# mrinmoy-iitg/SM_HPSS_MTL

Hardware: AMD Instinct MI355X
Metric: clips/sec HPSS+MTL-CNN fwd (1s@16kHz) (higher is better)
Workload: dtype f32

## Files before the change

sm_hpss_mtl_amd/build.py:

```python
from __future__ import annotations

import os
import subprocess
import sys
from concurrent.futures import ThreadPoolExecutor

HERE = os.path.dirname(os.path.abspath(__file__))
CSRC = os.path.join(HERE, "csrc")
OBJ = os.path.join(CSRC, "build")
LIB = os.path.join(HERE, "libsmh.so")
ARCH = "gfx950"
FLAGS = ["--offload-arch=" + ARCH, "-O3", "-fPIC", "-std=c++17", "-Wall", "-Wno-unused-function"]
EXTRA_FLAGS = {"smh_median_split.hip": ["-fno-honor-nans"], "smh_train.hip": ["-munsafe-fp-atomics"],
               "smh_tcn.hip": ["-fno-honor-nans"], "smh_tcn_bf16.hip": ["-fno-honor-nans"],
               "smh_train_bf16.hip": ["-munsafe-fp-atomics", "-fno-honor-nans"]}


def _sources():
    return sorted(f for f in os.listdir(CSRC) if f.endswith(".hip"))


def _headers_mtime():
    hs = [os.path.join(CSRC, f) for f in os.listdir(CSRC) if f.endswith(".h")]
    hs.append(os.path.join(HERE, "..", "include", "smh.h"))
    return max(os.path.getmtime(h) for h in hs)


LAB = False


def _compile(src: str, force: bool) -> str:
    obj = os.path.join(OBJ, src[:-4] + ".o")
    srcp = os.path.join(CSRC, src)
    if not force and os.path.exists(obj) and os.path.getmtime(obj) >= max(os.path.getmtime(srcp), _headers_mtime()):
        return obj
    cmd = ["hipcc", *FLAGS, *(["-DSMH_LAB"] if LAB else []), *EXTRA_FLAGS.get(src, []), "-c", srcp, "-o", obj]
    r = subprocess.run(cmd, capture_output=True, text=True)
    if r.returncode != 0:
        raise RuntimeError("hipcc failed for %s:\n%s\n%s" % (src, r.stdout, r.stderr))
    return obj


def build(force: bool = False, verbose: bool = True) -> str:
    os.makedirs(OBJ, exist_ok=True)
    srcs = _sources()
    with ThreadPoolExecutor(max_workers=min(6, len(srcs))) as ex:
        objs = list(ex.map(lambda s: _compile(s, force), srcs))
    if force or not os.path.exists(LIB) or any(os.path.getmtime(o) > os.path.getmtime(LIB) for o in objs):
        cmd = ["hipcc", "--offload-arch=" + ARCH, "-shared", "-fPIC", "-o", LIB, *objs]
        r = subprocess.run(cmd, capture_output=True, text=True)
        if r.returncode != 0:
            raise RuntimeError("link failed:\n%s\n%s" % (r.stdout, r.stderr))
    if verbose:
        print("built", LIB, "from", len(srcs), "HIP sources")
    return LIB


if __name__ == "__main__":
    LAB = "--lab" in sys.argv
    build(force="--force" in sys.argv or LAB)
```

sm_hpss_mtl_amd/csrc/smh_median.hip:

```cpp
#include <cstdlib>

#include "smh_median_kernel.h"
#include "smh_median_split.h"

namespace smh_median {

const Entry kPairs[] = {
    SMH_MEDIAN_E2(21, 11) SMH_MEDIAN_E2(17, 17)
    SMH_MEDIAN_E2(11, 11) SMH_MEDIAN_E2(11, 21) SMH_MEDIAN_E2(11, 31) SMH_MEDIAN_E2(11, 41) SMH_MEDIAN_E2(11, 51)
    SMH_MEDIAN_E2(21, 21) SMH_MEDIAN_E2(21, 31) SMH_MEDIAN_E2(21, 41) SMH_MEDIAN_E2(21, 51)
    SMH_MEDIAN_E2(31, 11) SMH_MEDIAN_E2(31, 21) SMH_MEDIAN_E2(31, 31) SMH_MEDIAN_E2(31, 41) SMH_MEDIAN_E2(31, 51)
    SMH_MEDIAN_E2(41, 11) SMH_MEDIAN_E2(41, 21) SMH_MEDIAN_E2(41, 31) SMH_MEDIAN_E2(41, 41) SMH_MEDIAN_E2(41, 51)
    SMH_MEDIAN_E2(51, 11) SMH_MEDIAN_E2(51, 21) SMH_MEDIAN_E2(51, 31) SMH_MEDIAN_E2(51, 41) SMH_MEDIAN_E2(51, 51)};

KernelFn find_pair_kernel(int lh, int lp) {
    for (const Entry &e : kPairs)
        if (e.lh == lh && e.lp == lp) return e.fn;
    return nullptr;
}

}

namespace {

// ... 93 lines not shown
    int bh = 0, bp = 0;
    for (int nsh = lh ? 1 : 0; nsh <= (lh ? 4 : 0); ++nsh) {
        if (lh && nsh > 1 && nt < 2 * lh * nsh) break;
        for (int nsp = lp ? 1 : 0; nsp <= (lp ? 6 : 0); ++nsp) {
            if (lp && nsp > 1 && K < 2 * lp * nsp) break;
            if (waves(K, nsh) + waves(nt, nsp) > maxwaves) continue;
            const long ch = lh ? (long)((nt + nsh - 1) / nsh + lh) * (lh + 6) : 0;
            const long cp = lp ? (long)((K + nsp - 1) / nsp + lp) * (lp + 6) : 0;
            const long c = ch > cp ? ch : cp;
            if (best < 0 || c < best) best = c, bh = nsh, bp = nsp;
        }
    }
    if (best < 0) return false;
    if (const char *ev = getenv("SMH_MEDIAN_SEG")) {
        int a = 0, b = 0;
        if (sscanf(ev, "%d,%d", &a, &b) == 2 && (!lh || a >= 1) && (!lp || b >= 1) &&
            waves(K, lh ? a : 0) + waves(nt, lp ? b : 0) <= maxwaves)
            bh = lh ? a : 0, bp = lp ? b : 0;
    }
    p->nsh = bh, p->nsp = bp, p->nwh = waves(K, bh), p->nwp = waves(nt, bp);
    return true;
}

int launch_small(const float *S, int B, int K, int T, int w, int along_t, float *out, hipStream_t st) {
    const size_t total = (size_t)B * K * T;
    const int bs = 256;
    hipLaunchKernelGGL(median_small_kernel, dim3((unsigned)((total + bs - 1) / bs)), dim3(bs), 0, st, S, out, K, T, w,
                       along_t, total);
    return smh::launch_status("median_small_kernel");
}

enum Family { kFamCopy = 0, kFamSmall = 1, kFamSplit = 2, kFamPersist = 3, kFamDeleteInsert = 4, kFamTwoSingles = 5 };
struct Route {
    int family, layout;
    Plan plan;
    KernelFn fn;
    const SplitEntry *se;
    const PersistEntry *pe;
    int n_cu;
};

int launch_route(int B, int K, int T, int lh, int lp, int harm_tmajor, Route *r) {
    *r = Route{};
    r->layout = harm_tmajor;
    r->fn = (lh && lp) ? find_pair_kernel(lh, lp) : find_single_kernel(lh, lp);
    if (!r->fn) return smh::set_error(SMH_E_INVALID, "no median kernel for (l_harm,l_perc)=(%d,%d)", lh, lp);
    Plan p;
    int rc = make_plan(K, T, lh, lp, &p);
    if (rc) return rc;
    static const bool no_split = getenv("SMH_MEDIAN_NOSPLIT") != nullptr;
    bool want_persist = (lh > 17 || lp > 17);
    if (const char *ev = getenv("SMH_MEDIAN_PERSIST")) want_persist = atoi(ev) != 0;
    int pthreads = 512;
    if (const char *ev = getenv("SMH_MEDIAN_PTHREADS")) pthreads = atoi(ev);
    if (const PersistEntry *pe = (no_split || !want_persist || !(lh && lp)) ? nullptr : find_persist_kernel(lh, lp, pthreads)) {
        static int n_cu = 0;
        if (n_cu == 0) {
            int dev = 0;
            SMH_CHECK_HIP(hipGetDevice(&dev));
            SMH_CHECK_HIP(hipDeviceGetAttribute(&n_cu, hipDeviceAttributeMultiprocessorCount, dev));
        }
        const int tile_bytes = persist_tile_bytes(K, T);
        const int g = T & 63;
        const bool conflict_free = (T & 1) || (g % 4 == 2);
        Plan q = p;
        if (p.ntiles == 1 && conflict_free && 2 * tile_bytes <= smh::kLdsBytesPerCU && B >= 2 * n_cu &&
            make_split_roles(K, T, lh, lp, pe->threads / 64, &q)) {
            r->family = kFamPersist, r->plan = q, r->pe = pe, r->n_cu = n_cu;
            return SMH_OK;
        }
    }
    if (const SplitEntry *se = no_split ? nullptr : find_split_kernel(lh, lp)) {
        Plan q = p;
        if (make_split_roles(K, p.TT, lh, lp, se->threads / 64, &q)) {
            r->family = kFamSplit, r->plan = q, r->se = se;
            return SMH_OK;
        }
    }
    if (harm_tmajor == 2) r->layout = 1;
    r->family = kFamDeleteInsert, r->plan = p;
    return SMH_OK;
}

int launch_routed(const Route &r, const float *S, int B, int K, int T, float *harm, float *perc, hipStream_t st) {
    if (r.family == kFamPersist) {
        const Plan &q = r.plan;
        const int lds = 2 * persist_tile_bytes(K, T);
        SMH_CHECK_HIP(hipFuncSetAttribute((const void *)r.pe->fn, hipFuncAttributeMaxDynamicSharedMemorySize, lds));
        hipLaunchKernelGGL(r.pe->fn, dim3(r.n_cu), dim3((q.nwh + q.nwp) * 64), lds, st, S, harm, perc, B, K, T, q.nsh,
                           q.nsp, q.nwh, r.layout);
        return smh::launch_status("hpss_median_persist_kernel");
    }
    if (r.family == kFamSplit) {
        const Plan &q = r.plan;
        SMH_CHECK_HIP(hipFuncSetAttribute((const void *)r.se->fn, hipFuncAttributeMaxDynamicSharedMemorySize, (int)q.lds));
        SMH_CHECK_HIP(hipFuncSetAttribute((const void *)r.se->fn_dma, hipFuncAttributeMaxDynamicSharedMemorySize, (int)q.lds));
        dim3 grid(q.ntiles, B), block((q.nwh + q.nwp) * 64);
        const bool probe_noload = smh::probe_env("SMH_MEDIAN_PROBE_NOLOAD") != nullptr;
        const char *ev = getenv("SMH_MEDIAN_DMA_STAGE");
        const size_t clip_bytes = (size_t)K * T * sizeof(float);
        const uintptr_t s0 = reinterpret_cast<uintptr_t>(S);
        const size_t align = (s0 % 16 == 0 && clip_bytes % 16 == 0) ? 16 : (s0 % 8 == 0 && clip_bytes % 8 == 0) ? 8 : 4;
        const bool dma = !(ev && atoi(ev) == 0) && !probe_noload && q.ntiles == 1 && q.TT >= T && s0 % 4 == 0 &&
                         ((T & 1) || ((T & 63) % 4 == 2)) && dma_stage_bytes(clip_bytes, align) <= q.lds;
        hipLaunchKernelGGL(dma ? r.se->fn_dma : r.se->fn, grid, block, q.lds, st, S, harm, perc, K, T, q.TT, dma ? T : q.stride, q.nsh,
                           q.nsp, q.nwh, r.layout, probe_noload ? 1.f : -__builtin_inff(), __builtin_inff(), nullptr, nullptr, 0);
        return smh::launch_status("hpss_median_split_kernel");
    }
    const Plan &p = r.plan;
    SMH_CHECK_HIP(hipFuncSetAttribute((const void *)r.fn, hipFuncAttributeMaxDynamicSharedMemorySize, (int)p.lds));
    dim3 grid(p.ntiles, B), block((p.nwh + p.nwp) * 64);
    hipLaunchKernelGGL(r.fn, grid, block, p.lds, st, S, harm, perc, K, T, p.TT, p.stride, p.nsh, p.nsp, p.nwh,
                       r.layout, -__builtin_inff(), __builtin_inff());
    return smh::launch_status("hpss_median_kernel");
}

int launch(const float *S, int B, int K, int T, int lh, int lp, float *harm, float *perc, hipStream_t st,
           int harm_tmajor = 0, int *written = nullptr) {
    if (written) *written = harm_tmajor;
    Route r;
    int rc = launch_route(B, K, T, lh, lp, harm_tmajor, &r);
    if (rc) return rc;
    if (written) *written = r.layout;
    return launch_routed(r, S, B, K, T, harm, perc, st);
}

int check_args(const void *S, int B, int K, int T, int w, const char *name) {
    SMH_REQUIRE(S != nullptr || B == 0, "%s: null input", name);
    SMH_REQUIRE(B >= 0 && K >= 1 && T >= 1, "%s: bad shape B=%d K=%d T=%d", name, B, K, T);
    SMH_REQUIRE(w >= 1 && w <= SMH_MAX_MEDIAN && (w & 1), "%s: window must be odd in [1,%d], got %d", name,
                SMH_MAX_MEDIAN, w);
    SMH_REQUIRE(B <= 65535, "%s: B=%d exceeds the grid limit; split the batch", name, B);
    return SMH_OK;
}

bool fast_ok(int n, int w) { return w >= 3 && w / 2 + 4 < n; }

bool pair_fused(int K, int T, int lh, int lp) { return fast_ok(T, lh) && fast_ok(K, lp) && find_pair_kernel(lh, lp); }

int hpss_route(int B, int K, int T, int lh, int lp, int want_tmajor, Route *r) {
    if (pair_fused(K, T, lh, lp)) return launch_route(B, K, T, lh, lp, want_tmajor, r);
    *r = Route{};
    r->family = kFamTwoSingles;
    return SMH_OK;
}

int time_route(int B, int K, int T, int lh, Route *r) {
    if (lh == 1 || !fast_ok(T, lh)) {
        *r = Route{};
        r->family = lh == 1 ? kFamCopy : kFamSmall;
        return SMH_OK;
    }
    return launch_route(B, K, T, lh, 0, 0, r);
}

int time_ex_route(int B, int K, int T, int lh, int harm_layout, Route *r) {
    if (lh == 1 || !fast_ok(T, lh) || harm_layout == 0) return time_route(B, K, T, lh, r);
    return launch_route(B, K, T, lh, 0, harm_layout, r);
}

}

namespace smh_median {
int rag_tile_frames(int K, int lh, int lp, int *stride) {
    static const bool no_split = getenv("SMH_MEDIAN_NOSPLIT") != nullptr;
    if (no_split || !(lh && lp) || !find_split_kernel(lh, lp)) return 0;
    const int hh = lh / 2;
    const int budget_words = (smh::kLdsBytesPerCU / 2 - 1024) / 4;
    int maxcols = budget_words / K;
    if ((maxcols & 1) == 0) maxcols -= 1;
    int TT = (maxcols - 2 * hh) & ~3;
    if (TT < 2 * hh + 8) return 0;
    if (stride) *stride = (TT + 2 * hh) | 1;
    return TT;
}

int launch_rag(const float *d_S, float *d_harm, float *d_perc, int K, int lh, int lp, const smh_rag::Clip *d_clips,
               const smh_rag::Item *d_items, int n_items, hipStream_t st) {
    if (n_items <= 0) return SMH_OK;
    int stride = 0;
    const int TT = rag_tile_frames(K, lh, lp, &stride);
    const SplitEntry *se = TT ? find_split_kernel(lh, lp) : nullptr;
    Plan q;
    if (!se || !make_split_roles(K, TT, lh, lp, se->threads / 64, &q))
        return smh::set_error(SMH_E_INVALID, "ragged medians: no block-split kernel for (l_harm,l_perc)=(%d,%d), K=%d", lh, lp, K);
    const size_t lds = (size_t)K * stride * sizeof(float);
    SMH_CHECK_HIP(hipFuncSetAttribute((const void *)se->fn, hipFuncAttributeMaxDynamicSharedMemorySize, (int)lds));
    const unsigned grid = (unsigned)(8 * (((long long)n_items + 7) / 8));
    hipLaunchKernelGGL(se->fn, dim3(grid), dim3((q.nwh + q.nwp) * 64), lds, st, d_S, d_harm, d_perc, K, 0, TT, stride, q.nsh, q.nsp,
                       q.nwh, 2, -__builtin_inff(), __builtin_inff(), d_clips, d_items, n_items);
    return smh::launch_status("hpss_median_split_kernel (ragged)");
}

int launch_hpss(const float *S, int B, int K, int T, int lh, int lp, float *harm, float *perc, int want_tmajor,
                hipStream_t st) {
    Route r;
    int rc = hpss_route(B, K, T, lh, lp, want_tmajor, &r);
    if (rc) return rc;
    rc = r.family == kFamTwoSingles ? smh_hpss_median_f32(nullptr, S, B, K, T, lh, lp, harm, perc, (void *)st)
                                    : launch_routed(r, S, B, K, T, harm, perc, st);
    return rc ? rc : r.layout;
}

bool blocked_harm_ok(int K, int T, int lh, int lp) {
    static const bool no_split = getenv("SMH_MEDIAN_NOSPLIT") != nullptr;
    if (no_split || !pair_fused(K, T, lh, lp)) return false;
    const SplitEntry *se = find_split_kernel(lh, lp);
    Plan p, q;
    return se && make_plan(K, T, lh, lp, &p) == SMH_OK && make_split_roles(K, p.TT, lh, lp, se->threads / 64, &q);
}
}

extern "C" int smh_median_time_f32(const smh_ctx *, const float *d_S, int B, int K, int T, int l_harm, float *d_harm,
                                   void *stream) {
    int rc = check_args(d_S, B, K, T, l_harm, "smh_median_time_f32");
    if (rc) return rc;
    SMH_REQUIRE(d_harm || B == 0, "smh_median_time_f32: null output");
    if (B == 0) return SMH_OK;
    hipStream_t st = (hipStream_t)stream;
    Route r;
    rc = time_route(B, K, T, l_harm, &r);
    if (rc) return rc;
    if (r.family == kFamCopy) {
        SMH_CHECK_HIP(hipMemcpyAsync(d_harm, d_S, (size_t)B * K * T * sizeof(float), hipMemcpyDeviceToDevice, st));
        return SMH_OK;
    }
    if (r.family == kFamSmall) return launch_small(d_S, B, K, T, l_harm, 1, d_harm, st);
    return launch_routed(r, d_S, B, K, T, d_harm, nullptr, st);
}

extern "C" int smh_median_time_ex_f32(const smh_ctx *, const float *d_S, int B, int K, int T, int l_harm, float *d_harm,
                                      int harm_layout, void *stream) {
    int rc = check_args(d_S, B, K, T, l_harm, "smh_median_time_ex_f32");
    if (rc) return rc;
    SMH_REQUIRE(harm_layout >= 0 && harm_layout <= 2, "smh_median_time_ex_f32: harm_layout must be 0, 1 or 2");
    SMH_REQUIRE(d_harm || B == 0, "smh_median_time_ex_f32: null output");
    if (B == 0) return harm_layout;
    Route r;
    rc = time_ex_route(B, K, T, l_harm, harm_layout, &r);
    if (rc) return rc;
    if (r.family == kFamCopy || r.family == kFamSmall) {
        rc = smh_median_time_f32(nullptr, d_S, B, K, T, l_harm, d_harm, stream);
        return rc ? rc : 0;
    }
    rc = launch_routed(r, d_S, B, K, T, d_harm, nullptr, (hipStream_t)stream);
    return rc ? rc : r.layout;
}

extern "C" int smh_median_freq_f32(const smh_ctx *, const float *d_S, int B, int K, int T, int l_perc, float *d_perc,
                                   void *stream) {
    int rc = check_args(d_S, B, K, T, l_perc, "smh_median_freq_f32");
    if (rc) return rc;
    SMH_REQUIRE(d_perc || B == 0, "smh_median_freq_f32: null output");
    if (B == 0) return SMH_OK;
    hipStream_t st = (hipStream_t)stream;
    if (l_perc == 1) {
        SMH_CHECK_HIP(hipMemcpyAsync(d_perc, d_S, (size_t)B * K * T * sizeof(float), hipMemcpyDeviceToDevice, st));
        return SMH_OK;
    }
    if (!fast_ok(K, l_perc)) return launch_small(d_S, B, K, T, l_perc, 0, d_perc, st);
    return launch(d_S, B, K, T, 0, l_perc, nullptr, d_perc, st);
}

extern "C" int smh_hpss_median_f32(const smh_ctx *, const float *d_S, int B, int K, int T, int l_harm, int l_perc,
                                   float *d_harm, float *d_perc, void *stream) {
    int rc = check_args(d_S, B, K, T, l_harm, "smh_hpss_median_f32");
    if (rc) return rc;
    rc = check_args(d_S, B, K, T, l_perc, "smh_hpss_median_f32");
    if (rc) return rc;
    SMH_REQUIRE((d_harm && d_perc) || B == 0, "smh_hpss_median_f32: null output");
    if (B == 0) return SMH_OK;
    Route r;
// ... 45 lines not shown
```

sm_hpss_mtl_amd/csrc/smh_median_split.h:

```cpp
#pragma once
#include <cstdint>
#include <type_traits>
#include <utility>

#include "smh_median_kernel.h"
#include "smh_rag.h"

namespace smh_median {

template <int W>
struct SplitTraits {
    static constexpr int H = W / 2;
    static constexpr int lo(int s) { return s - H - 1 > 0 ? s - H - 1 : 0; }
    static constexpr int hi(int s) { return s - 1 < H ? s - 1 : H; }
    static constexpr int off(int s) {
        int o = 0;
        for (int r = 1; r < s; ++r) o += hi(r) - lo(r) + 1;
        return o;
    }
    static constexpr int HIST = off(W);
};

template <int B, int E, typename F>
__device__ __forceinline__ void static_for(F &&f) {
    if constexpr (B < E) {
        f(std::integral_constant<int, B>{});
        static_for<B + 1, E>(f);
    }
}
template <int B, int E, typename F>
__device__ __forceinline__ void static_for_down(F &&f) {
    if constexpr (B < E) {
        f(std::integral_constant<int, E - 1>{});
        static_for_down<B, E - 1>(f);
    }
}

template <bool HasBelow, bool HasAbove>
__device__ __forceinline__ float insert_slot(float below, float x, float above) {
    if constexpr (HasBelow && HasAbove) return med3(below, x, above);
    else if constexpr (HasBelow) return fmaxf(below, x);
    else if constexpr (HasAbove) return fminf(x, above);
    else return x;
}

template <int W>
__device__ __forceinline__ void build_history(const float (&e)[W], float (&h)[SplitTraits<W>::HIST]) {
    using Tr = SplitTraits<W>;
    static_for<1, W>([&](auto sc) {
        constexpr int s = decltype(sc)::value;
        const float x = e[W - s];
        static_for<Tr::lo(s), Tr::hi(s) + 1>([&](auto ic) {
            constexpr int i = decltype(ic)::value;
            constexpr bool has_below = i - 1 >= 0;
            constexpr bool has_above = i <= s - 2;
            constexpr int po = Tr::off(s > 1 ? s - 1 : 1), pl = Tr::lo(s > 1 ? s - 1 : 1);
            const float below = has_below ? h[has_below ? po + (i - 1) - pl : 0] : 0.f;
            const float above = has_above ? h[has_above ? po + i - pl : 0] : 0.f;
            h[Tr::off(s) + i - Tr::lo(s)] = insert_slot<has_below, has_above>(below, x, above);
        });
    });
}

template <int W, int ES, int STORE>
__device__ __forceinline__ void split_median_walk(const float *line, int es_rt, int p0, int n_out, int n_steps, int n,
                                                  char *obase, unsigned boff, unsigned ostep) {
    using Tr = SplitTraits<W>;
    constexpr int H = W / 2;
    const int es = ES > 0 ? ES : es_rt;
    float e[W];
    float h[Tr::HIST];
    float pre[H + 1];

    const int plast = p0 + n_out - 1 + H;
    auto load_block = [&](int q0) {
        const int lo = p0 - H + q0;
        const bool interior = (lo >= 0) & (lo + W <= n) & (lo + W - 1 <= plast);
        if (__all(interior)) {
            const float *src = line + lo * es;
            static_for<0, W>([&](auto uc) { e[decltype(uc)::value] = src[decltype(uc)::value * es]; });
        } else {
            static_for<0, W>([&](auto uc) {
                const int pos = min(lo + decltype(uc)::value, plast);
                e[decltype(uc)::value] = line[reflect_hi(reflect_lo(pos), n) * es];
            });
        }
    };
    unsigned off = boff;
    auto emit = [&](int j, float v, bool guard) {
        if (!guard || j < n_out) {
            float *dst = reinterpret_cast<float *>(obase + off);
#ifdef SMH_NT_STORES
            if constexpr (STORE == kStridedStream) __builtin_nontemporal_store(v, dst);
            else *dst = v;
#else
            *dst = v;
#endif
        }
        off += ostep;
    };
    int n_min = n_out;
#pragma unroll
    for (int o = 32; o >= 1; o >>= 1) n_min = min(n_min, __shfl_xor(n_min, o, 64));

    auto forward = [&](auto fast_c, int j0) {
        constexpr bool FAST = decltype(fast_c)::value;
        static_for<0, W>([&](auto pc) {
            constexpr int p = decltype(pc)::value;
            constexpr int b = p + 1, a = W - 1 - p;
            {
                static_for_down<Tr::lo(b), Tr::hi(b) + 1>([&](auto ic) {
                    constexpr int i = decltype(ic)::value;
                    constexpr bool has_below = i - 1 >= 0;
                    constexpr bool has_above = i <= b - 2;
                    const float below = has_below ? pre[has_below ? i - 1 : 0] : 0.f;
                    const float above = has_above ? pre[i] : 0.f;
                    pre[i] = insert_slot<has_below, has_above>(below, e[p], above);
                });
                constexpr int i_lo = (H + 1 - b) > 0 ? (H + 1 - b) : 0;
                constexpr int i_hi = a < H + 1 ? a : H + 1;
                constexpr int ao = Tr::off(a > 0 ? a : 1), al = Tr::lo(a > 0 ? a : 1);
                float r = 0.f;
                static_for<i_lo, i_hi + 1>([&](auto ic) {
                    constexpr int i = decltype(ic)::value;
                    float t;
                    if constexpr (i == 0) t = pre[H];
                    else if constexpr (H - i < 0) t = h[ao + (i - 1) - al];
                    else t = fmaxf(h[ao + (i - 1) - al], pre[H - i]);
                    r = (i == i_lo) ? t : fminf(r, t);
                });
                emit(j0 + p, r, !FAST);
            }
        });
    };

    load_block(0);
    build_history<W>(e, h);
    {
        constexpr int po = Tr::off(W - 1), pl = Tr::lo(W - 1);
        emit(0, med3(h[po + (H - 1) - pl], e[0], h[po + H - pl]), false);
    }
    for (int j0 = 1; j0 < n_steps; j0 += W) {
        load_block(j0 + W - 1);
        if (j0 + W <= n_min) forward(std::true_type{}, j0);
        else forward(std::false_type{}, j0);
        if (j0 + W < n_steps) build_history<W>(e, h);
    }
}

template <int W>
__device__ __forceinline__ void build_history_b(const float (&e)[W - 1], float (&h)[SplitTraits<W>::HIST]) {
    using Tr = SplitTraits<W>;
    static_for<1, W>([&](auto sc) {
        constexpr int s = decltype(sc)::value;
        const float x = e[W - 1 - s];
        static_for<Tr::lo(s), Tr::hi(s) + 1>([&](auto ic) {
            constexpr int i = decltype(ic)::value;
            constexpr bool has_below = i - 1 >= 0;
            constexpr bool has_above = i <= s - 2;
            constexpr int po = Tr::off(s > 1 ? s - 1 : 1), pl = Tr::lo(s > 1 ? s - 1 : 1);
            const float below = has_below ? h[has_below ? po + (i - 1) - pl : 0] : 0.f;
            const float above = has_above ? h[has_above ? po + i - pl : 0] : 0.f;
            h[Tr::off(s) + i - Tr::lo(s)] = insert_slot<has_below, has_above>(below, x, above);
        });
    });
}

template <int W, int ES>
__device__ __forceinline__ void split_median_walk_blocked(const float *line, int p0, int n_out, int n_steps, int n,
                                                          char *obase, unsigned gk16, unsigned kofs) {
    using Tr = SplitTraits<W>;
    constexpr int H = W / 2, BK = W - 1;
    float e[BK];
    float h[Tr::HIST];
    float pre[H + 1];
    const int plast = p0 + n_out - 1 + H;
    auto load_block = [&](int q0) {
        const int lo = p0 - H + q0;
        const bool interior = (lo >= 0) & (lo + BK <= n) & (lo + BK - 1 <= plast);
        if (__all(interior)) {
            const float *src = line + lo * ES;
            static_for<0, BK>([&](auto uc) { e[decltype(uc)::value] = src[decltype(uc)::value * ES]; });
        } else {
            static_for<0, BK>([&](auto uc) {
                const int pos = min(lo + decltype(uc)::value, plast);
                e[decltype(uc)::value] = line[reflect_hi(reflect_lo(pos), n) * ES];
            });
        }
    };
    load_block(0);
    build_history_b<W>(e, h);
    for (int j0 = 0; j0 < n_steps; j0 += BK) {
        load_block(j0 + BK);
        float o4[4];
        static_for<0, BK>([&](auto pc) {
            constexpr int p = decltype(pc)::value;
            constexpr int b = p + 1, a = BK - p;
            static_for_down<Tr::lo(b), Tr::hi(b) + 1>([&](auto ic) {
                constexpr int i = decltype(ic)::value;
                constexpr bool has_below = i - 1 >= 0;
                constexpr bool has_above = i <= b - 2;
                const float below = has_below ? pre[has_below ? i - 1 : 0] : 0.f;
                const float above = has_above ? pre[i] : 0.f;
                pre[i] = insert_slot<has_below, has_above>(below, e[p], above);
            });
            constexpr int i_lo = (H + 1 - b) > 0 ? (H + 1 - b) : 0;
            constexpr int i_hi = a < H + 1 ? a : H + 1;
            constexpr int ao = Tr::off(a), al = Tr::lo(a);
            float r = 0.f;
            static_for<i_lo, i_hi + 1>([&](auto ic) {
                constexpr int i = decltype(ic)::value;
                float t;
                if constexpr (i == 0) t = pre[H];
                else if constexpr (H - i < 0) t = h[ao + (i - 1) - al];
                else t = fmaxf(h[ao + (i - 1) - al], pre[H - i]);
                r = (i == i_lo) ? t : fminf(r, t);
            });
            o4[p & 3] = r;
            if constexpr ((p & 3) == 3 || p == BK - 1) {
                constexpr int cnt = (p & 3) + 1, pf = p - (p & 3);
                const int j = j0 + pf, t = p0 + j;
                char *dst = obase + (unsigned)(t >> 4) * gk16 + kofs + (unsigned)(t & 15) * 4u;
                if (cnt == 4 && (t & 3) == 0 && j + 3 < n_out) {
                    float4u v = {o4[0], o4[1], o4[2], o4[3]};
                    *reinterpret_cast<float4u *>(dst) = v;
                } else {
#pragma unroll
                    for (int c = 0; c < cnt; ++c) {
                        const int tc = t + c;
                        if (j + c < n_out)
                            *reinterpret_cast<float *>(obase + (unsigned)(tc >> 4) * gk16 + kofs + (unsigned)(tc & 15) * 4u) = o4[c];
                    }
                }
            }
        });
        if (j0 + BK < n_steps) build_history_b<W>(e, h);
    }
}

__device__ __forceinline__ int stage_clip_dma(const char *src, int bytes, char *dst, int wave, int nwaves, int lane) {
    const int mis = (int)(reinterpret_cast<uintptr_t>(src) & 15);
    src -= mis;
    const int nchunks = (bytes + mis + 15) >> 4;
    for (int i = wave; i * 64 < nchunks; i += nwaves) {
        const int c = i * 64 + lane;
        if (c < nchunks)
            __builtin_amdgcn_global_load_lds(
                (const __attribute__((address_space(1))) void *)(src + (size_t)c * 16),
                (__attribute__((address_space(3))) void *)(dst + i * 1024), 16, 0, 0);
    }
    return mis;
}
__host__ __device__ constexpr size_t dma_stage_bytes(size_t bytes, size_t align) { return (bytes + (16 - align) + 15) & ~(size_t)15; }

template <int LH, int LP>
struct SplitCfg {
    static constexpr int kMaxW = LH > LP ? LH : LP;
    static constexpr int kThreads = kMaxW <= 17 ? 512 : 384;
    static constexpr int kWavesPerSimd = kMaxW <= 17 ? 4 : 3;
    static constexpr int kFlatBatch = kMaxW <= 17 ? 20 : 27;
};

template <int LH, int LP, bool DMA = false>
__global__ void __launch_bounds__((SplitCfg<LH, LP>::kThreads), (SplitCfg<LH, LP>::kWavesPerSimd))
hpss_median_split_kernel(const float *__restrict__ S, float *__restrict__ harm, float *__restrict__ perc, int K, int T,
                         int TT, int stride, int nsh, int nsp, int nwh, int harm_tmajor, float probe, float,
                         const smh_rag::Clip *__restrict__ rag, const smh_rag::Item *__restrict__ items, int n_items) {
    extern __shared__ __attribute__((aligned(16))) float tile_lds[];
    const float *tile = tile_lds;
    constexpr int HH = LH / 2;
    int b = blockIdx.y, tile_i = blockIdx.x;
    size_t spec_off, harm_off;
    if (rag) {
        const unsigned total = (unsigned)n_items, per_xcd = (total + 7u) >> 3;
        const unsigned j = blockIdx.x >> 3, n = (blockIdx.x & 7u) * per_xcd + j;
        if (j >= per_xcd || n >= total) return;
        const smh_rag::Item item = items[n];
        b = item.clip, tile_i = item.tile;
        T = rag[b].T;
        spec_off = (size_t)rag[b].spec_off, harm_off = (size_t)rag[b].harm_off;
    } else {
        spec_off = (size_t)b * K * T;
        harm_off = harm_tmajor == 2 ? (size_t)b * ((T + 15) >> 4) * K * 16 : spec_off;
    }
    const int t0 = tile_i * TT;
    const int t1 = min(T, t0 + TT);
    const int c0 = max(0, t0 - HH), c1 = min(T, t1 + HH);
    const int ncols = c1 - c0;
    const float *Sb = S + spec_off;
    const int wave = threadIdx.x >> 6, lane = threadIdx.x & 63;
    const int nwaves = blockDim.x >> 6;

    constexpr int kFlatBatch = SplitCfg<LH, LP>::kFlatBatch;
    if constexpr (DMA) {
        const int mis = stage_clip_dma(reinterpret_cast<const char *>(Sb), K * T * 4, reinterpret_cast<char *>(tile_lds), wave, nwaves, lane);
        tile = reinterpret_cast<const float *>(reinterpret_cast<const char *>(tile_lds) + mis);
        asm volatile("s_waitcnt vmcnt(0)" ::: "memory");
    } else if (probe > 0.f) {
        for (int i = threadIdx.x; i < K * stride; i += blockDim.x) tile_lds[i] = (float)((i * 2654435761u) >> 8) * (1.0f / 16777216.f);
    } else if (TT >= T && ((K * T) & 1) == 0 && K * T <= kFlatBatch * 2 * (int)blockDim.x) {
        const int n2 = (K * T) >> 1;
        const float2v *src = reinterpret_cast<const float2v *>(Sb);
        const unsigned magic = 0xFFFFFFFFu / (unsigned)T + 1u;
        const int extra = stride - T;
        float2v v[kFlatBatch];
#pragma unroll
        for (int r = 0; r < kFlatBatch; ++r) {
            const int idx = r * (int)blockDim.x + (int)threadIdx.x;
            v[r] = __builtin_nontemporal_load(src + min(idx, n2 - 1));
        }
#pragma unroll
        for (int r = 0; r < kFlatBatch; ++r) {
            const int idx = r * (int)blockDim.x + (int)threadIdx.x;
            if (idx < n2) {
                const unsigned g = 2u * (unsigned)idx;
                const unsigned k0 = __umulhi(g, magic), k1 = __umulhi(g + 1u, magic);
                tile_lds[g + k0 * extra] = v[r].x;
                tile_lds[g + 1u + k1 * extra] = v[r].y;
            }
        }
    } else if (((T | c0 | ncols) & 1) == 0 && ncols <= 128) {
        constexpr int kRowBatch = 6;
        const int n2 = ncols >> 1;
        for (int k0 = wave; k0 < K; k0 += nwaves * kRowBatch) {
            float2v v[kRowBatch];
#pragma unroll
            for (int r = 0; r < kRowBatch; ++r) {
                const int k = min(k0 + r * nwaves, K - 1);
                v[r] = __builtin_nontemporal_load(reinterpret_cast<const float2v *>(Sb + (size_t)k * T + c0) +
                                                  min(lane, n2 - 1));
            }
#pragma unroll
            for (int r = 0; r < kRowBatch; ++r) {
                const int k = k0 + r * nwaves;
                if (k < K && lane < n2) {
                    tile_lds[k * stride + 2 * lane] = v[r].x;
                    tile_lds[k * stride + 2 * lane + 1] = v[r].y;
                }
            }
        }
    } else {
        constexpr int kRowBatch = 6;
        for (int k0 = wave; k0 < K; k0 += nwaves * kRowBatch) {
            for (int cb = 0; cb < ncols; cb += 64) {
                float v[kRowBatch];
                const int c = cb + lane;
#pragma unroll
                for (int r = 0; r < kRowBatch; ++r) {
                    const int k = min(k0 + r * nwaves, K - 1);
                    v[r] = __builtin_nontemporal_load(Sb + (size_t)k * T + c0 + min(c, ncols - 1));
                }
#pragma unroll
                for (int r = 0; r < kRowBatch; ++r) {
                    const int k = k0 + r * nwaves;
                    if (k < K && c < ncols) tile_lds[k * stride + c] = v[r];
                }
            }
        }
    }
    __syncthreads();

    const int nt = t1 - t0;
    if (wave < nwh) {
        if constexpr (LH > 0) {
            const int id = wave * 64 + lane;
            if (id < K * nsh) {
                const int sg = id / K, k = id - sg * K;
                const int seglen = (nt + nsh - 1) / nsh;
                const int ts = t0 + sg * seglen;
                const int te = min(t1, ts + seglen);
                if (ts < te) {
                    const float *row = tile + k * stride - c0;
                    char *ob = reinterpret_cast<char *>(harm + harm_off);
                    if (harm_tmajor == 2)
                        split_median_walk_blocked<LH, 1>(row, ts, te - ts, seglen, T, ob, (unsigned)K * 64u, (unsigned)k * 64u);
                    else if (harm_tmajor)
                        split_median_walk<LH, 1, kStridedPlain>(row, 1, ts, te - ts, seglen, T, ob,
                                                                (unsigned)(ts * K + k) * 4u, (unsigned)K * 4u);
                    else
                        split_median_walk<LH, 1, kStridedPlain>(row, 1, ts, te - ts, seglen, T, ob,
                                                                (unsigned)(k * T + ts) * 4u, 4u);
                }
            }
        }
    } else {
        if constexpr (LP > 0) {
            const int id = (wave - nwh) * 64 + lane;
            if (id < nt * nsp) {
                const int sg = id / nt, tt = id - sg * nt;
                const int seglen = (K + nsp - 1) / nsp;
                const int ks = sg * seglen;
                const int ke = min(K, ks + seglen);
                if (ks < ke) {
                    const float *col = tile + (t0 + tt - c0);
                    split_median_walk<LP, 0, kStridedStream>(col, stride, ks, ke - ks, seglen, K,
                                                             reinterpret_cast<char *>(perc + spec_off),
                                                             (unsigned)(ks * T + t0 + tt) * 4u, (unsigned)T * 4u);
                }
            }
        }
    }
}

__host__ __device__ constexpr int persist_tile_bytes(int K, int T) { return ((K * T * 4 + 16) + 1023) & ~1023; }

template <int LH, int LP, int THREADS>
__global__ void __launch_bounds__(THREADS, (THREADS / 256))
hpss_median_persist_kernel(const float *__restrict__ S, float *__restrict__ harm, float *__restrict__ perc, int B, int K,
                           int T, int nsh, int nsp, int nwh, int harm_tmajor) {
    extern __shared__ __attribute__((aligned(16))) char lds[];
    const int tile_bytes = persist_tile_bytes(K, T);
    const int wave = threadIdx.x >> 6, lane = threadIdx.x & 63;
    const int nwaves = blockDim.x >> 6;
    const size_t clip_bytes = (size_t)K * T * 4;

    auto issue_load = [&](int b, int buf) {
        stage_clip_dma(reinterpret_cast<const char *>(S) + (size_t)b * clip_bytes, (int)clip_bytes, lds + buf * tile_bytes, wave, nwaves, lane);
    };

    int b = blockIdx.x;
    if (b >= B) return;
    issue_load(b, 0);
    for (int it = 0; b < B; b += gridDim.x, ++it) {
        const int cur = it & 1;
        asm volatile("s_waitcnt vmcnt(0)" ::: "memory");
        __syncthreads();
        if (b + (int)gridDim.x < B) issue_load(b + gridDim.x, cur ^ 1);
        const int mis = (int)((reinterpret_cast<uintptr_t>(S) + (size_t)b * clip_bytes) & 15);
        const float *tile = reinterpret_cast<const float *>(lds + cur * tile_bytes + mis);
        if (wave < nwh) {
            const int id = wave * 64 + lane;
            if (id < K * nsh) {
                const int sg = id / K, k = id - sg * K;
                const int seglen = (T + nsh - 1) / nsh;
                const int ts = sg * seglen;
                const int te = min(T, ts + seglen);
                if (ts < te) {
                    const float *row = tile + k * T;
                    char *ob = reinterpret_cast<char *>(harm + (size_t)b * K * T);
                    if (harm_tmajor == 2)
                        split_median_walk_blocked<LH, 1>(row, ts, te - ts, seglen, T,
                                                         reinterpret_cast<char *>(harm + (size_t)b * ((T + 15) >> 4) * K * 16),
                                                         (unsigned)K * 64u, (unsigned)k * 64u);
                    else if (harm_tmajor)
                        split_median_walk<LH, 1, kStridedPlain>(row, 1, ts, te - ts, seglen, T, ob,
                                                                (unsigned)(ts * K + k) * 4u, (unsigned)K * 4u);
                    else
                        split_median_walk<LH, 1, kStridedPlain>(row, 1, ts, te - ts, seglen, T, ob,
                                                                (unsigned)(k * T + ts) * 4u, 4u);
                }
            }
        } else {
            const int id = (wave - nwh) * 64 + lane;
            if (id < T * nsp) {
                const int sg = id / T, tt = id - sg * T;
                const int seglen = (K + nsp - 1) / nsp;
                const int ks = sg * seglen;
                const int ke = min(K, ks + seglen);
                if (ks < ke)
                    split_median_walk<LP, 0, kStridedStream>(tile + tt, T, ks, ke - ks, seglen, K,
                                                             reinterpret_cast<char *>(perc + (size_t)b * K * T),
                                                             (unsigned)(ks * T + tt) * 4u, (unsigned)T * 4u);
            }
        }
    }
}

using PersistFn = void (*)(const float *, float *, float *, int, int, int, int, int, int, int);
struct PersistEntry {
    int lh, lp, threads;
    PersistFn fn;
};
const PersistEntry *find_persist_kernel(int lh, int lp, int threads);

constexpr int kSplitMaxWindow = 21;

using SplitFn = void (*)(const float *, float *, float *, int, int, int, int, int, int, int, int, float, float,
                         const smh_rag::Clip *, const smh_rag::Item *, int);
struct SplitEntry {
    int lh, lp, threads;
    SplitFn fn, fn_dma;
};
const SplitEntry *find_split_kernel(int lh, int lp);

}
```

sm_hpss_mtl_amd/csrc/smh_median_split.hip:

```cpp
#include "smh_median_split.h"

namespace smh_median {

#define SMH_SPLIT_E2(a, b) {a, b, SplitCfg<a, b>::kThreads, hpss_median_split_kernel<a, b>, hpss_median_split_kernel<a, b, true>},
#define SMH_SPLIT_SINGLE(w) SMH_SPLIT_E2(w, 0) SMH_SPLIT_E2(0, w)

const SplitEntry kSplit[] = {
    SMH_SPLIT_E2(21, 11) SMH_SPLIT_E2(17, 17) SMH_SPLIT_E2(11, 11) SMH_SPLIT_E2(11, 21) SMH_SPLIT_E2(21, 21)
    SMH_SPLIT_SINGLE(3) SMH_SPLIT_SINGLE(5) SMH_SPLIT_SINGLE(7) SMH_SPLIT_SINGLE(9) SMH_SPLIT_SINGLE(11)
    SMH_SPLIT_SINGLE(13) SMH_SPLIT_SINGLE(15) SMH_SPLIT_SINGLE(17) SMH_SPLIT_SINGLE(19) SMH_SPLIT_SINGLE(21)};

const SplitEntry *find_split_kernel(int lh, int lp) {
    for (const SplitEntry &e : kSplit)
        if (e.lh == lh && e.lp == lp) return &e;
    return nullptr;
}

#define SMH_PERSIST_E3(a, b, t) {a, b, t, hpss_median_persist_kernel<a, b, t>},
#define SMH_PERSIST_E2(a, b) SMH_PERSIST_E3(a, b, 512) SMH_PERSIST_E3(a, b, 768)
const PersistEntry kPersist[] = {SMH_PERSIST_E2(21, 11) SMH_PERSIST_E2(17, 17) SMH_PERSIST_E2(11, 11)
                                 SMH_PERSIST_E2(11, 21) SMH_PERSIST_E2(21, 21) SMH_PERSIST_E3(17, 17, 1024)};

const PersistEntry *find_persist_kernel(int lh, int lp, int threads) {
    for (const PersistEntry &e : kPersist)
        if (e.lh == lh && e.lp == lp && e.threads == threads) return &e;
    return nullptr;
}

}
```

Before: 2.777 million.

## Add wave-uniform median walk with scalar edges, whole-row interior test and vector tail stores

Adds a new WALK variant of the split/persist median kernels and makes it the default, keeping the old path behind SMH_MEDIAN_WALK=0. When the whole row is resident, the interior check no longer clips at the segment end. Boundary loads use wave-uniform scalar indices when all lanes share the same segment. The blocked-layout harmonic walk gets specialised partial-block tails and float4 stores when the segment is 4-aligned, and the per-walk wave shuffle reduction is dropped. The aim is less divergent boundary handling, fewer scalar stores and less wasted tail work, at the cost of more template instances and more complex control flow.

Result: no change. 2.806 million (median of 6 runs) (+1.1%).

```diff
diff --git a/sm_hpss_mtl_amd/build.py b/sm_hpss_mtl_amd/build.py
--- a/sm_hpss_mtl_amd/build.py
+++ b/sm_hpss_mtl_amd/build.py
@@ -11,7 +11,8 @@
 LIB = os.path.join(HERE, "libsmh.so")
 ARCH = "gfx950"
 FLAGS = ["--offload-arch=" + ARCH, "-O3", "-fPIC", "-std=c++17", "-Wall", "-Wno-unused-function"]
-EXTRA_FLAGS = {"smh_median_split.hip": ["-fno-honor-nans"], "smh_train.hip": ["-munsafe-fp-atomics"],
+EXTRA_FLAGS = {"smh_median_split.hip": ["-fno-honor-nans"], "smh_median_split_walk0.hip": ["-fno-honor-nans"],
+               "smh_train.hip": ["-munsafe-fp-atomics"],
                "smh_tcn.hip": ["-fno-honor-nans"], "smh_tcn_bf16.hip": ["-fno-honor-nans"],
                "smh_train_bf16.hip": ["-munsafe-fp-atomics", "-fno-honor-nans"]}
 
diff --git a/sm_hpss_mtl_amd/csrc/smh_median.hip b/sm_hpss_mtl_amd/csrc/smh_median.hip
--- a/sm_hpss_mtl_amd/csrc/smh_median.hip
+++ b/sm_hpss_mtl_amd/csrc/smh_median.hip
@@ -199,19 +199,28 @@
     return SMH_OK;
 }
 
+static bool old_walk() {
+    const char *ev = getenv("SMH_MEDIAN_WALK");
+    return ev && atoi(ev) == 0;
+}
+
 int launch_routed(const Route &r, const float *S, int B, int K, int T, float *harm, float *perc, hipStream_t st) {
+    const bool walk0 = old_walk();
     if (r.family == kFamPersist) {
         const Plan &q = r.plan;
         const int lds = 2 * persist_tile_bytes(K, T);
-        SMH_CHECK_HIP(hipFuncSetAttribute((const void *)r.pe->fn, hipFuncAttributeMaxDynamicSharedMemorySize, lds));
-        hipLaunchKernelGGL(r.pe->fn, dim3(r.n_cu), dim3((q.nwh + q.nwp) * 64), lds, st, S, harm, perc, B, K, T, q.nsh,
+        const PersistFn pfn = walk0 ? find_persist_kernel(r.pe->lh, r.pe->lp, r.pe->threads, true)->fn : r.pe->fn;
+        SMH_CHECK_HIP(hipFuncSetAttribute((const void *)pfn, hipFuncAttributeMaxDynamicSharedMemorySize, lds));
+        hipLaunchKernelGGL(pfn, dim3(r.n_cu), dim3((q.nwh + q.nwp) * 64), lds, st, S, harm, perc, B, K, T, q.nsh,
                            q.nsp, q.nwh, r.layout);
         return smh::launch_status("hpss_median_persist_kernel");
     }
     if (r.family == kFamSplit) {
         const Plan &q = r.plan;
-        SMH_CHECK_HIP(hipFuncSetAttribute((const void *)r.se->fn, hipFuncAttributeMaxDynamicSharedMemorySize, (int)q.lds));
-        SMH_CHECK_HIP(hipFuncSetAttribute((const void *)r.se->fn_dma, hipFuncAttributeMaxDynamicSharedMemorySize, (int)q.lds));
+        const SplitEntry *se = walk0 ? find_split_kernel(r.se->lh, r.se->lp, true) : r.se;
+        const SplitFn fn = se->fn, fn_dma = se->fn_dma;
+        SMH_CHECK_HIP(hipFuncSetAttribute((const void *)fn, hipFuncAttributeMaxDynamicSharedMemorySize, (int)q.lds));
+        SMH_CHECK_HIP(hipFuncSetAttribute((const void *)fn_dma, hipFuncAttributeMaxDynamicSharedMemorySize, (int)q.lds));
         dim3 grid(q.ntiles, B), block((q.nwh + q.nwp) * 64);
         const bool probe_noload = smh::probe_env("SMH_MEDIAN_PROBE_NOLOAD") != nullptr;
         const char *ev = getenv("SMH_MEDIAN_DMA_STAGE");
@@ -220,7 +229,7 @@
         const size_t align = (s0 % 16 == 0 && clip_bytes % 16 == 0) ? 16 : (s0 % 8 == 0 && clip_bytes % 8 == 0) ? 8 : 4;
         const bool dma = !(ev && atoi(ev) == 0) && !probe_noload && q.ntiles == 1 && q.TT >= T && s0 % 4 == 0 &&
                          ((T & 1) || ((T & 63) % 4 == 2)) && dma_stage_bytes(clip_bytes, align) <= q.lds;
-        hipLaunchKernelGGL(dma ? r.se->fn_dma : r.se->fn, grid, block, q.lds, st, S, harm, perc, K, T, q.TT, dma ? T : q.stride, q.nsh,
+        hipLaunchKernelGGL(dma ? fn_dma : fn, grid, block, q.lds, st, S, harm, perc, K, T, q.TT, dma ? T : q.stride, q.nsh,
                            q.nsp, q.nwh, r.layout, probe_noload ? 1.f : -__builtin_inff(), __builtin_inff(), nullptr, nullptr, 0);
         return smh::launch_status("hpss_median_split_kernel");
     }
@@ -302,9 +311,10 @@
     if (!se || !make_split_roles(K, TT, lh, lp, se->threads / 64, &q))
         return smh::set_error(SMH_E_INVALID, "ragged medians: no block-split kernel for (l_harm,l_perc)=(%d,%d), K=%d", lh, lp, K);
     const size_t lds = (size_t)K * stride * sizeof(float);
-    SMH_CHECK_HIP(hipFuncSetAttribute((const void *)se->fn, hipFuncAttributeMaxDynamicSharedMemorySize, (int)lds));
+    const SplitFn fn = old_walk() ? find_split_kernel(lh, lp, true)->fn : se->fn;
+    SMH_CHECK_HIP(hipFuncSetAttribute((const void *)fn, hipFuncAttributeMaxDynamicSharedMemorySize, (int)lds));
     const unsigned grid = (unsigned)(8 * (((long long)n_items + 7) / 8));
-    hipLaunchKernelGGL(se->fn, dim3(grid), dim3((q.nwh + q.nwp) * 64), lds, st, d_S, d_harm, d_perc, K, 0, TT, stride, q.nsh, q.nsp,
+    hipLaunchKernelGGL(fn, dim3(grid), dim3((q.nwh + q.nwp) * 64), lds, st, d_S, d_harm, d_perc, K, 0, TT, stride, q.nsh, q.nsp,
                        q.nwh, 2, -__builtin_inff(), __builtin_inff(), d_clips, d_items, n_items);
     return smh::launch_status("hpss_median_split_kernel (ragged)");
 }
diff --git a/sm_hpss_mtl_amd/csrc/smh_median_split.h b/sm_hpss_mtl_amd/csrc/smh_median_split.h
--- a/sm_hpss_mtl_amd/csrc/smh_median_split.h
+++ b/sm_hpss_mtl_amd/csrc/smh_median_split.h
@@ -62,9 +62,24 @@
     });
 }
 
-template <int W, int ES, int STORE>
+#ifndef SMH_WALK_PARTS
+#define SMH_WALK_PARTS 7
+#endif
+constexpr bool kWalkTails = SMH_WALK_PARTS & 1, kWalkWhole = SMH_WALK_PARTS & 2, kWalkStores = SMH_WALK_PARTS & 4,
+               kWalkScalarEdges = SMH_WALK_PARTS & 8;
+struct WaveWalk {
+    bool uni;
+    int p0, n_out, plast;
+};
+template <int H>
+__device__ __forceinline__ WaveWalk wave_walk(int p0, int n_out) {
+    const int sp0 = __builtin_amdgcn_readfirstlane(p0), sn = __builtin_amdgcn_readfirstlane(n_out);
+    return {__all((p0 == sp0) & (n_out == sn)) != 0, sp0, sn, sp0 + sn - 1 + H};
+}
+
+template <int W, int ES, int STORE, int WALK = 1>
 __device__ __forceinline__ void split_median_walk(const float *line, int es_rt, int p0, int n_out, int n_steps, int n,
-                                                  char *obase, unsigned boff, unsigned ostep) {
+                                                  char *obase, unsigned boff, unsigned ostep, bool whole = false) {
     using Tr = SplitTraits<W>;
     constexpr int H = W / 2;
     const int es = ES > 0 ? ES : es_rt;
@@ -73,12 +88,20 @@
     float pre[H + 1];
 
     const int plast = p0 + n_out - 1 + H;
+    WaveWalk ww = {false, 0, 0, 0};
+    if constexpr (WALK) ww = wave_walk<H>(p0, n_out);
     auto load_block = [&](int q0) {
         const int lo = p0 - H + q0;
-        const bool interior = (lo >= 0) & (lo + W <= n) & (lo + W - 1 <= plast);
+        const bool interior = (lo >= 0) & (lo + W <= n) & ((WALK && kWalkWhole && whole) | (lo + W - 1 <= plast));
         if (__all(interior)) {
             const float *src = line + lo * es;
             static_for<0, W>([&](auto uc) { e[decltype(uc)::value] = src[decltype(uc)::value * es]; });
+        } else if (WALK && kWalkScalarEdges && ww.uni) {
+            const int slo = ww.p0 - H + q0;
+            static_for<0, W>([&](auto uc) {
+                const int pos = min(slo + decltype(uc)::value, ww.plast);
+                e[decltype(uc)::value] = line[reflect_hi(reflect_lo(pos), n) * es];
+            });
         } else {
             static_for<0, W>([&](auto uc) {
                 const int pos = min(lo + decltype(uc)::value, plast);
@@ -100,8 +123,10 @@
         off += ostep;
     };
     int n_min = n_out;
-#pragma unroll
-    for (int o = 32; o >= 1; o >>= 1) n_min = min(n_min, __shfl_xor(n_min, o, 64));
+    if constexpr (!WALK) {
+#pragma unroll
+        for (int o = 32; o >= 1; o >>= 1) n_min = min(n_min, __shfl_xor(n_min, o, 64));
+    }
 
     auto forward = [&](auto fast_c, int j0) {
         constexpr bool FAST = decltype(fast_c)::value;
@@ -238,6 +263,106 @@
     }
 }
 
+template <int W, int ES>
+__device__ __forceinline__ void split_median_walk_blocked_tails(const float *line, int p0, int n_out, int n_steps, int n,
+                                                                char *obase, unsigned gk16, unsigned kofs, bool whole) {
+    using Tr = SplitTraits<W>;
+    constexpr int H = W / 2, BK = W - 1, NG = (BK + 3) / 4;
+    constexpr bool TAILS = kWalkTails && W <= 17;
+    float e[BK];
+    float h[Tr::HIST];
+    float pre[H + 1];
+    const int plast = p0 + n_out - 1 + H;
+    const WaveWalk ww = wave_walk<H>(p0, n_out);
+    const bool vec_ok = kWalkStores && BK % 4 == 0 && ww.uni && (ww.p0 & 3) == 0;
+    auto load_block = [&](auto nec, int q0) {
+        constexpr int NE = decltype(nec)::value;
+        const int lo = p0 - H + q0;
+        const bool interior = (lo >= 0) & (lo + NE <= n) & ((kWalkWhole && whole) | (lo + NE - 1 <= plast));
+        if (__all(interior)) {
+            const float *src = line + lo * ES;
+            static_for<0, NE>([&](auto uc) { e[decltype(uc)::value] = src[decltype(uc)::value * ES]; });
+        } else if (kWalkScalarEdges && ww.uni) {
+            const int slo = ww.p0 - H + q0;
+            static_for<0, NE>([&](auto uc) {
+                const int pos = min(slo + decltype(uc)::value, ww.plast);
+                e[decltype(uc)::value] = line[reflect_hi(reflect_lo(pos), n) * ES];
+            });
+        } else {
+            static_for<0, NE>([&](auto uc) {
+                const int pos = min(lo + decltype(uc)::value, plast);
+                e[decltype(uc)::value] = line[reflect_hi(reflect_lo(pos), n) * ES];
+            });
+        }
+    };
+    auto block = [&](auto gc, int j0) {
+        constexpr int NS = 4 * decltype(gc)::value < BK ? 4 * decltype(gc)::value : BK;
+        load_block(std::integral_constant<int, NS>{}, j0 + BK);
+        const bool all_live = vec_ok && j0 + NS <= ww.n_out;
+        float o4[4];
+        static_for<0, NS>([&](auto pc) {
+            constexpr int p = decltype(pc)::value;
+            constexpr int b = p + 1, a = BK - p;
+            static_for_down<Tr::lo(b), Tr::hi(b) + 1>([&](auto ic) {
+                constexpr int i = decltype(ic)::value;
+                constexpr bool has_below = i - 1 >= 0;
+                constexpr bool has_above = i <= b - 2;
+                const float below = has_below ? pre[has_below ? i - 1 : 0] : 0.f;
+                const float above = has_above ? pre[i] : 0.f;
+                pre[i] = insert_slot<has_below, has_above>(below, e[p], above);
+            });
+            constexpr int i_lo = (H + 1 - b) > 0 ? (H + 1 - b) : 0;
+            constexpr int i_hi = a < H + 1 ? a : H + 1;
+            constexpr int ao = Tr::off(a), al = Tr::lo(a);
+            float r = 0.f;
+            static_for<i_lo, i_hi + 1>([&](auto ic) {
+                constexpr int i = decltype(ic)::value;
+                float t;
+                if constexpr (i == 0) t = pre[H];
+                else if constexpr (H - i < 0) t = h[ao + (i - 1) - al];
+                else t = fmaxf(h[ao + (i - 1) - al], pre[H - i]);
+                r = (i == i_lo) ? t : fminf(r, t);
+            });
+            o4[p & 3] = r;
+            if constexpr ((p & 3) == 3 || p == NS - 1) {
+                constexpr int cnt = (p & 3) + 1, pf = p - (p & 3);
+                if (cnt == 4 && all_live) {
+                    const int st = ww.p0 + j0 + pf;
+                    const unsigned grp = (unsigned)(st >> 4) * gk16 + (unsigned)(st & 15) * 4u;
+                    float4u v = {o4[0], o4[1], o4[2], o4[3]};
+                    *reinterpret_cast<float4u *>(obase + (grp + kofs)) = v;
+                } else {
+                    const int j = j0 + pf, t = p0 + j;
+                    if (cnt == 4 && (t & 3) == 0 && j + 3 < n_out) {
+                        float4u v = {o4[0], o4[1], o4[2], o4[3]};
+                        *reinterpret_cast<float4u *>(obase + ((unsigned)(t >> 4) * gk16 + kofs + (unsigned)(t & 15) * 4u)) = v;
+                    } else {
+#pragma unroll
+                        for (int c = 0; c < cnt; ++c) {
+                            const int tc = t + c;
+                            if (j + c < n_out)
+                                *reinterpret_cast<float *>(obase + ((unsigned)(tc >> 4) * gk16 + kofs + (unsigned)(tc & 15) * 4u)) = o4[c];
+                        }
+                    }
+                }
+            }
+        });
+    };
+    load_block(std::integral_constant<int, BK>{}, 0);
+    build_history_b<W>(e, h);
+    int j0 = 0;
+    for (; n_steps - j0 > (TAILS ? 4 * (NG - 1) : 0); j0 += BK) {
+        block(std::integral_constant<int, NG>{}, j0);
+        if (j0 + BK < n_steps) build_history_b<W>(e, h);
+    }
+    if (TAILS && j0 < n_steps) {
+        const int g = (n_steps - j0 + 3) >> 2;
+        static_for<1, NG>([&](auto gc) {
+            if (g == decltype(gc)::value) block(gc, j0);
+        });
+    }
+}
+
 __device__ __forceinline__ int stage_clip_dma(const char *src, int bytes, char *dst, int wave, int nwaves, int lane) {
     const int mis = (int)(reinterpret_cast<uintptr_t>(src) & 15);
     src -= mis;
@@ -261,7 +386,7 @@
     static constexpr int kFlatBatch = kMaxW <= 17 ? 20 : 27;
 };
 
-template <int LH, int LP, bool DMA = false>
+template <int LH, int LP, bool DMA = false, int WALK = 1>
 __global__ void __launch_bounds__((SplitCfg<LH, LP>::kThreads), (SplitCfg<LH, LP>::kWavesPerSimd))
 hpss_median_split_kernel(const float *__restrict__ S, float *__restrict__ harm, float *__restrict__ perc, int K, int T,
                          int TT, int stride, int nsh, int nsp, int nwh, int harm_tmajor, float probe, float,
@@ -372,14 +497,18 @@
                 if (ts < te) {
                     const float *row = tile + k * stride - c0;
                     char *ob = reinterpret_cast<char *>(harm + harm_off);
-                    if (harm_tmajor == 2)
-                        split_median_walk_blocked<LH, 1>(row, ts, te - ts, seglen, T, ob, (unsigned)K * 64u, (unsigned)k * 64u);
-                    else if (harm_tmajor)
-                        split_median_walk<LH, 1, kStridedPlain>(row, 1, ts, te - ts, seglen, T, ob,
-                                                                (unsigned)(ts * K + k) * 4u, (unsigned)K * 4u);
+                    const bool whole = ncols == T;
+                    if (harm_tmajor == 2) {
+                        if constexpr (WALK)
+                            split_median_walk_blocked_tails<LH, 1>(row, ts, te - ts, seglen, T, ob, (unsigned)K * 64u, (unsigned)k * 64u, whole);
+                        else
+                            split_median_walk_blocked<LH, 1>(row, ts, te - ts, seglen, T, ob, (unsigned)K * 64u, (unsigned)k * 64u);
+                    } else if (harm_tmajor)
+                        split_median_walk<LH, 1, kStridedPlain, WALK>(row, 1, ts, te - ts, seglen, T, ob,
+                                                                      (unsigned)(ts * K + k) * 4u, (unsigned)K * 4u, whole);
                     else
-                        split_median_walk<LH, 1, kStridedPlain>(row, 1, ts, te - ts, seglen, T, ob,
-                                                                (unsigned)(k * T + ts) * 4u, 4u);
+                        split_median_walk<LH, 1, kStridedPlain, WALK>(row, 1, ts, te - ts, seglen, T, ob,
+                                                                      (unsigned)(k * T + ts) * 4u, 4u, whole);
                 }
             }
         }
@@ -393,9 +522,9 @@
                 const int ke = min(K, ks + seglen);
                 if (ks < ke) {
                     const float *col = tile + (t0 + tt - c0);
-                    split_median_walk<LP, 0, kStridedStream>(col, stride, ks, ke - ks, seglen, K,
-                                                             reinterpret_cast<char *>(perc + spec_off),
-                                                             (unsigned)(ks * T + t0 + tt) * 4u, (unsigned)T * 4u);
+                    split_median_walk<LP, 0, kStridedStream, WALK>(col, stride, ks, ke - ks, seglen, K,
+                                                                   reinterpret_cast<char *>(perc + spec_off),
+                                                                   (unsigned)(ks * T + t0 + tt) * 4u, (unsigned)T * 4u, true);
                 }
             }
         }
@@ -404,7 +533,7 @@
 
 __host__ __device__ constexpr int persist_tile_bytes(int K, int T) { return ((K * T * 4 + 16) + 1023) & ~1023; }
 
-template <int LH, int LP, int THREADS>
+template <int LH, int LP, int THREADS, int WALK = 1>
 __global__ void __launch_bounds__(THREADS, (THREADS / 256))
 hpss_median_persist_kernel(const float *__restrict__ S, float *__restrict__ harm, float *__restrict__ perc, int B, int K,
                            int T, int nsh, int nsp, int nwh, int harm_tmajor) {
@@ -438,16 +567,18 @@
                 if (ts < te) {
                     const float *row = tile + k * T;
                     char *ob = reinterpret_cast<char *>(harm + (size_t)b * K * T);
-                    if (harm_tmajor == 2)
-                        split_median_walk_blocked<LH, 1>(row, ts, te - ts, seglen, T,
-                                                         reinterpret_cast<char *>(harm + (size_t)b * ((T + 15) >> 4) * K * 16),
-                                                         (unsigned)K * 64u, (unsigned)k * 64u);
-                    else if (harm_tmajor)
-                        split_median_walk<LH, 1, kStridedPlain>(row, 1, ts, te - ts, seglen, T, ob,
-                                                                (unsigned)(ts * K + k) * 4u, (unsigned)K * 4u);
+                    if (harm_tmajor == 2) {
+                        char *ob2 = reinterpret_cast<char *>(harm + (size_t)b * ((T + 15) >> 4) * K * 16);
+                        if constexpr (WALK)
+                            split_median_walk_blocked_tails<LH, 1>(row, ts, te - ts, seglen, T, ob2, (unsigned)K * 64u, (unsigned)k * 64u, true);
+                        else
+                            split_median_walk_blocked<LH, 1>(row, ts, te - ts, seglen, T, ob2, (unsigned)K * 64u, (unsigned)k * 64u);
+                    } else if (harm_tmajor)
+                        split_median_walk<LH, 1, kStridedPlain, WALK>(row, 1, ts, te - ts, seglen, T, ob,
+                                                                      (unsigned)(ts * K + k) * 4u, (unsigned)K * 4u, true);
                     else
-                        split_median_walk<LH, 1, kStridedPlain>(row, 1, ts, te - ts, seglen, T, ob,
-                                                                (unsigned)(k * T + ts) * 4u, 4u);
+                        split_median_walk<LH, 1, kStridedPlain, WALK>(row, 1, ts, te - ts, seglen, T, ob,
+                                                                      (unsigned)(k * T + ts) * 4u, 4u, true);
                 }
             }
         } else {
@@ -458,9 +589,9 @@
                 const int ks = sg * seglen;
                 const int ke = min(K, ks + seglen);
                 if (ks < ke)
-                    split_median_walk<LP, 0, kStridedStream>(tile + tt, T, ks, ke - ks, seglen, K,
-                                                             reinterpret_cast<char *>(perc + (size_t)b * K * T),
-                                                             (unsigned)(ks * T + tt) * 4u, (unsigned)T * 4u);
+                    split_median_walk<LP, 0, kStridedStream, WALK>(tile + tt, T, ks, ke - ks, seglen, K,
+                                                                   reinterpret_cast<char *>(perc + (size_t)b * K * T),
+                                                                   (unsigned)(ks * T + tt) * 4u, (unsigned)T * 4u, true);
             }
         }
     }
@@ -471,7 +602,8 @@
     int lh, lp, threads;
     PersistFn fn;
 };
-const PersistEntry *find_persist_kernel(int lh, int lp, int threads);
+const PersistEntry *find_persist_kernel(int lh, int lp, int threads, bool walk0 = false);
+const PersistEntry *find_persist_kernel_walk0(int lh, int lp, int threads);
 
 constexpr int kSplitMaxWindow = 21;
 
@@ -481,6 +613,21 @@
     int lh, lp, threads;
     SplitFn fn, fn_dma;
 };
-const SplitEntry *find_split_kernel(int lh, int lp);
-
-}
+const SplitEntry *find_split_kernel(int lh, int lp, bool walk0 = false);
+const SplitEntry *find_split_kernel_walk0(int lh, int lp);
+
+#define SMH_SPLIT_E2(a, b, w) {a, b, SplitCfg<a, b>::kThreads, hpss_median_split_kernel<a, b, false, w>, hpss_median_split_kernel<a, b, true, w>},
+#define SMH_SPLIT_SINGLE(x, w) SMH_SPLIT_E2(x, 0, w) SMH_SPLIT_E2(0, x, w)
+#define SMH_SPLIT_TABLE(w)                                                                                                       \
+                  \
+    SMH_SPLIT_E2(21, 11, w) SMH_SPLIT_E2(17, 17, w) SMH_SPLIT_E2(11, 11, w) SMH_SPLIT_E2(11, 21, w) SMH_SPLIT_E2(21, 21, w)      \
+                                                                                                             \
+    SMH_SPLIT_SINGLE(3, w) SMH_SPLIT_SINGLE(5, w) SMH_SPLIT_SINGLE(7, w) SMH_SPLIT_SINGLE(9, w) SMH_SPLIT_SINGLE(11, w)          \
+    SMH_SPLIT_SINGLE(13, w) SMH_SPLIT_SINGLE(15, w) SMH_SPLIT_SINGLE(17, w) SMH_SPLIT_SINGLE(19, w) SMH_SPLIT_SINGLE(21, w)
+#define SMH_PERSIST_E3(a, b, t, w) {a, b, t, hpss_median_persist_kernel<a, b, t, w>},
+#define SMH_PERSIST_E2(a, b, w) SMH_PERSIST_E3(a, b, 512, w) SMH_PERSIST_E3(a, b, 768, w)
+#define SMH_PERSIST_TABLE(w)                                                                                               \
+    SMH_PERSIST_E2(21, 11, w) SMH_PERSIST_E2(17, 17, w) SMH_PERSIST_E2(11, 11, w) SMH_PERSIST_E2(11, 21, w) SMH_PERSIST_E2(21, 21, w) \
+    SMH_PERSIST_E3(17, 17, 1024, w)
+
+}
diff --git a/sm_hpss_mtl_amd/csrc/smh_median_split.hip b/sm_hpss_mtl_amd/csrc/smh_median_split.hip
--- a/sm_hpss_mtl_amd/csrc/smh_median_split.hip
+++ b/sm_hpss_mtl_amd/csrc/smh_median_split.hip
@@ -2,26 +2,19 @@
 
 namespace smh_median {
 
-#define SMH_SPLIT_E2(a, b) {a, b, SplitCfg<a, b>::kThreads, hpss_median_split_kernel<a, b>, hpss_median_split_kernel<a, b, true>},
-#define SMH_SPLIT_SINGLE(w) SMH_SPLIT_E2(w, 0) SMH_SPLIT_E2(0, w)
+const SplitEntry kSplit[] = {SMH_SPLIT_TABLE(1)};
 
-const SplitEntry kSplit[] = {
-    SMH_SPLIT_E2(21, 11) SMH_SPLIT_E2(17, 17) SMH_SPLIT_E2(11, 11) SMH_SPLIT_E2(11, 21) SMH_SPLIT_E2(21, 21)
-    SMH_SPLIT_SINGLE(3) SMH_SPLIT_SINGLE(5) SMH_SPLIT_SINGLE(7) SMH_SPLIT_SINGLE(9) SMH_SPLIT_SINGLE(11)
-    SMH_SPLIT_SINGLE(13) SMH_SPLIT_SINGLE(15) SMH_SPLIT_SINGLE(17) SMH_SPLIT_SINGLE(19) SMH_SPLIT_SINGLE(21)};
-
-const SplitEntry *find_split_kernel(int lh, int lp) {
+const SplitEntry *find_split_kernel(int lh, int lp, bool walk0) {
+    if (walk0) return find_split_kernel_walk0(lh, lp);
     for (const SplitEntry &e : kSplit)
         if (e.lh == lh && e.lp == lp) return &e;
     return nullptr;
 }
 
-#define SMH_PERSIST_E3(a, b, t) {a, b, t, hpss_median_persist_kernel<a, b, t>},
-#define SMH_PERSIST_E2(a, b) SMH_PERSIST_E3(a, b, 512) SMH_PERSIST_E3(a, b, 768)
-const PersistEntry kPersist[] = {SMH_PERSIST_E2(21, 11) SMH_PERSIST_E2(17, 17) SMH_PERSIST_E2(11, 11)
-                                 SMH_PERSIST_E2(11, 21) SMH_PERSIST_E2(21, 21) SMH_PERSIST_E3(17, 17, 1024)};
+const PersistEntry kPersist[] = {SMH_PERSIST_TABLE(1)};
 
-const PersistEntry *find_persist_kernel(int lh, int lp, int threads) {
+const PersistEntry *find_persist_kernel(int lh, int lp, int threads, bool walk0) {
+    if (walk0) return find_persist_kernel_walk0(lh, lp, threads);
     for (const PersistEntry &e : kPersist)
         if (e.lh == lh && e.lp == lp && e.threads == threads) return &e;
     return nullptr;
diff --git a/sm_hpss_mtl_amd/csrc/smh_median_split_walk0.hip b/sm_hpss_mtl_amd/csrc/smh_median_split_walk0.hip
--- /dev/null
+++ b/sm_hpss_mtl_amd/csrc/smh_median_split_walk0.hip
@@ -0,0 +1,21 @@
+#include "smh_median_split.h"
+
+namespace smh_median {
+
+const SplitEntry kSplitWalk0[] = {SMH_SPLIT_TABLE(0)};
+
+const SplitEntry *find_split_kernel_walk0(int lh, int lp) {
+    for (const SplitEntry &e : kSplitWalk0)
+        if (e.lh == lh && e.lp == lp) return &e;
+    return nullptr;
+}
+
+const PersistEntry kPersistWalk0[] = {SMH_PERSIST_TABLE(0)};
+
+const PersistEntry *find_persist_kernel_walk0(int lh, int lp, int threads) {
+    for (const PersistEntry &e : kPersistWalk0)
+        if (e.lh == lh && e.lp == lp && e.threads == threads) return &e;
+    return nullptr;
+}
+
+}
```
